# edegens/ptype

Hardware: AMD Instinct MI355X
Metric: messages/sec (higher is better)
Workload: dtype int64; 1 GPU; model=calculator actor (Calculator.Multiply), global_batch=8388608, parallelism=actors sharded over 1 GPU(s), actors=131072, chunks=1, wire=v2, record_bytes=20, reply_bytes=9, client_batch=SoA (actor u32, A i64, B i64), hip_graph=True, steps_per_graph=1, placement=random, delivery=mailbox, mailbox_slots=131072, mailbox_ring_bytes=1344380288, mailbox_record_bytes=8

## Files before the change

### ptype_amd/csrc/hip/mailbox_sort_dev.hpp

```cpp
#pragma once
#include <algorithm>
#include <type_traits>
#include <vector>

#include "mailbox.hpp"
#include "mailbox_dev.hpp"
#include "route_common.hpp"
#include "sort_common.hpp"
#include "tune.hpp"

namespace ptype {

namespace {
constexpr uint32_t kCompactMark = 0x80000000u;
constexpr uint32_t kCompactLong = 0x80000000u;
constexpr int kOrdThreads = 512;
constexpr int kOrdK = 4;
constexpr int kOrdWin = kOrdThreads * kOrdK;
constexpr int kOrdWaves = kOrdThreads / kWave;
constexpr uint32_t kOrdStateMax = 4096;
}

constexpr uint32_t kGroupBlocks = 32;
constexpr uint32_t kNoSlot = 0xffffffffu;
constexpr uint32_t kSpillSlot = 0xfffffffeu;
constexpr uint32_t kRunSpilled = 0x80000000u;

template <int MODE>
__global__ __launch_bounds__(kST) void mbx_count_kernel(SortIn in, uint32_t log_s, uint32_t* __restrict__ hist,
                                                        uint32_t* __restrict__ gsum, uint32_t* __restrict__ rw) {
  __shared__ uint32_t cnt[kMboxSortMaxShards];
  const uint32_t S = 1u << log_s;
  const uint32_t v = virt_block(blockIdx.x, in.G);
  for (uint32_t s = threadIdx.x; s < S; s += kST) cnt[s] = 0;
  __syncthreads();
  const uint32_t t0 = v * in.tpb, t1 = min(t0 + in.tpb, in.tiles);
  uint32_t a[kSK];
  if (t0 < t1) load_actors(in, t0, a);
  for (uint32_t t = t0; t < t1; ++t) {
    int r[kSK];
    uint32_t mb[kSK];
    resolve_k<MODE>(in, a, r, mb);
    if (t + 1 < t1) load_actors(in, t + 1, a);
#pragma unroll
    for (int k = 0; k < kSK; ++k) {
      const int64_t i = tile_index(t, k);
      const bool ok = r[k] == in.rank_self && mb[k] < kMaxMbox;
      if (i < in.M) rw[i] = ok ? mb[k] : kNoSlot;
      if (ok) atomicAdd(&cnt[mb[k] & (S - 1)], 1u);
    }
  }
  __syncthreads();
  uint32_t* g = gsum + (size_t)(v / kGroupBlocks) * S;
  for (uint32_t s = threadIdx.x; s < S; s += kST) {
    const uint32_t c = cnt[s];
    hist[(size_t)v * S + s] = c;
    if (c) atomicAdd(&g[s], c);
  }
}

template <bool A2, bool MC>
__device__ __forceinline__ void load_routed(const SortIn& in, const uint32_t* __restrict__ rw, uint32_t t,
                                            uint32_t (&m)[kSK], int64_t (&x0)[kSK], int64_t (&x1)[kSK],
                                            int64_t (&x2)[kSK], uint32_t (&meth)[kSK]) {
#pragma unroll
  for (int k = 0; k < kSK; ++k) {
    const int64_t i = tile_index(t, k);
    const bool ok = i < in.M;
    m[k] = ok ? __builtin_nontemporal_load(rw + i) : kNoSlot;
    x0[k] = ok ? __builtin_nontemporal_load(in.a0 + i) : 0;
    x1[k] = ok && in.a1 ? __builtin_nontemporal_load(in.a1 + i) : 0;
    x2[k] = 0;
    if constexpr (A2) x2[k] = ok ? __builtin_nontemporal_load(in.a2 + i) : 0;
    meth[k] = in.method_uniform;
    if constexpr (MC) meth[k] = ok ? (uint32_t)in.mcol[i] : 0u;
  }
}

__host__ __device__ constexpr size_t scatter_lds_bytes(uint32_t S) { return (size_t)S * (16 + 4 * (kST / kWave)); }

template <bool A2, bool MC>
__global__ __launch_bounds__(kST) void mbx_scatter_kernel(SortIn in, MboxView mv, const uint32_t* __restrict__ hist,
                                                          const uint32_t* __restrict__ gsum,
                                                          uint32_t* __restrict__ rw,
                                                          uint32_t* __restrict__ sidx, uint32_t* __restrict__ tinfo,
                                                          ReplyView rv, bool spill, bool all_sidx) {
  extern __shared__ __align__(16) unsigned char smem_sc[];
  const uint32_t S = 1u << mv.log_s;
  unsigned long long* base = reinterpret_cast<unsigned long long*>(smem_sc);
  uint32_t* run = reinterpret_cast<uint32_t*>(base + S);
  uint32_t* room = run + S;
  uint32_t* wcnt_all = room + S;
  auto wcnt = [&](unsigned ww, uint32_t sh) -> uint32_t& { return wcnt_all[ww * S + sh]; };
  const uint64_t Q = 1ull << mv.log_q;
  const uint32_t v = virt_block(blockIdx.x, in.G);
  const unsigned w = threadIdx.x / kWave, lane = lane_id();
  const uint32_t g0 = v / kGroupBlocks, v0 = g0 * kGroupBlocks;
  for (uint32_t s = threadIdx.x; s < S; s += kST) {
    uint32_t p = 0;
    for (uint32_t g = 0; g < g0; ++g) p += gsum[(size_t)g * S + s];
    for (uint32_t u = v0; u < v; ++u) p += hist[(size_t)u * S + s];
    run[s] = p;
    const uint64_t tl = *ctr_tail(mv, s), hd = *ctr_head(mv, s);
    base[s] = tl;
    const uint64_t free = hd + Q > tl ? hd + Q - tl : 0;
    room[s] = (uint32_t)(free < 0xffffffffull ? free : 0xffffffffull);
  }
  unsigned long long n_enq = 0, n_ovf = 0, n_miss = 0, n_spill = 0;
  const uint32_t t0 = v * in.tpb, t1 = min(t0 + in.tpb, in.tiles);
  for (uint32_t t = t0; t < t1; ++t) {
    for (uint32_t s = lane; s < S; s += kWave) wcnt(w, s) = 0;
    uint32_t mb[kSK], meth[kSK];
    int64_t v0[kSK], v1[kSK], v2[kSK];
    load_routed<A2, MC>(in, rw, t, mb, v0, v1, v2, meth);
    uint32_t wr[kSK], sh[kSK];
#pragma unroll
    for (int k = 0; k < kSK; ++k) {
      const bool ok = mb[k] != kNoSlot;
      sh[k] = mb[k] & (S - 1);
      const uint64_t peers = match_bits(sh[k], mv.log_s, __ballot(ok));
      const unsigned below = mbcnt64(peers);
      const int leader = peers ? __builtin_ctzll(peers) : 0;
      unsigned old = 0;
      if (ok && below == 0) {
        old = wcnt(w, sh[k]);
        wcnt(w, sh[k]) = old + (unsigned)__popcll(peers);
      }
      wr[k] = (unsigned)__shfl((int)old, leader) + below;
    }
    __syncthreads();
    int sp = 0;
    for (uint32_t s = threadIdx.x; s < S; s += kST) {
      uint32_t rr = run[s];
#pragma unroll
      for (int ww = 0; ww < kST / kWave; ++ww) {
        const uint32_t c = wcnt(ww, s);
        wcnt(ww, s) = rr;
        rr += c;
      }
      run[s] = rr;
      sp |= rr > room[s];
    }
    bool tile_spill = false;
    if (spill) tile_spill = __syncthreads_or(sp) != 0;
    else __syncthreads();
    const bool wsidx = all_sidx || tile_spill;
#pragma unroll
    for (int k = 0; k < kSK; ++k) {
      const int64_t i = tile_index(t, k);
      if (i >= in.M) continue;
      const uint32_t origin = in.origin_base + (uint32_t)i;
      if (mb[k] == kNoSlot) {
        ++n_miss;
        if (wsidx) sidx[i] = kNoSlot;
        write_status(rv, origin, kStatusNoActor);
        continue;
      }
      const uint32_t off = wcnt(w, sh[k]) + wr[k];
      if (off >= room[sh[k]]) {
        if (spill) {
          ++n_spill;
          sidx[i] = kSpillSlot;
          continue;
        }
        ++n_ovf;
        if (wsidx) sidx[i] = kNoSlot;
        write_status(rv, origin, kStatusOverflow);
        continue;
      }
      const int64_t x0 = v0[k], x1 = v1[k], x2 = v2[k];
      const uint32_t mt = meth[k];
      const uint64_t slot = slot_at(mv, sh[k], base[sh[k]] + off);
      if (wsidx) sidx[i] = (uint32_t)slot;
      if (mt < 128u && fits_i32(x0) && fits_i32(x1) && x2 == 0) {
        *reinterpret_cast<u32x4*>(rec_a(mv, slot)) =
            u32x4{origin | kCompactMark, mb[k] | (mt << 24), (uint32_t)x0, (uint32_t)x1};
      } else {
        const uint32_t fl = x2 != 0 ? (uint32_t)kFlagA2 : 0u;
        *reinterpret_cast<u32x4*>(rec_a(mv, slot)) =
            u32x4{origin | kCompactMark, mb[k] | kCompactLong, (mt & 0xffffu) | (fl << 16), 0u};
        *reinterpret_cast<u32x4*>(rec_b(mv, slot)) =
            u32x4{(uint32_t)x0, (uint32_t)((uint64_t)x0 >> 32), (uint32_t)x1, (uint32_t)((uint64_t)x1 >> 32)};
        if (fl) mv.a2[slot] = x2;
      }
      ++n_enq;
    }
    if (tinfo) {
      for (uint32_t s = threadIdx.x; s < S; s += kST) {
        const uint32_t r0 = wcnt(0, s), rr = run[s];
        const uint32_t cc = r0 >= room[s] ? 0u : min(rr - r0, room[s] - r0);
        tinfo[(size_t)t * 2 * S + s] = (uint32_t)(base[s] + r0) + shard_rot(mv, s);
        tinfo[(size_t)t * 2 * S + S + s] = cc | (rr > room[s] ? kRunSpilled : 0u);
      }
    }
    __syncthreads();
  }
  block_add_stats(mv.stats, n_enq, kMbEnqueued, n_ovf, kMbOverflow, n_miss, kMbNoActor);
  if (spill) {
    __syncthreads();
    block_add_stats(mv.stats, n_spill, kMbSpilled, 0, -1, 0, -1);
  }
}

__host__ __device__ constexpr size_t onesweep_lds_bytes(uint32_t S) { return (size_t)S * (8 + 4 + 4 + 4 * (kST / kWave)); }

template <bool A2, bool MC, int SK = kSK>
__device__ __forceinline__ void load_cols(const SortIn& in, uint32_t t, int64_t (&v0)[SK], int64_t (&v1)[SK],
                                          int64_t (&v2)[SK], uint32_t (&meth)[SK]) {
#pragma unroll
  for (int k = 0; k < SK; ++k) {
    const int64_t i = tile_index<SK>(t, k);
    const bool ok = i < in.M;
    v0[k] = ok ? __builtin_nontemporal_load(in.a0 + i) : 0;
    v1[k] = ok && in.a1 ? __builtin_nontemporal_load(in.a1 + i) : 0;
    v2[k] = 0;
    if constexpr (A2) v2[k] = ok ? __builtin_nontemporal_load(in.a2 + i) : 0;
    meth[k] = in.method_uniform;
    if constexpr (MC) meth[k] = ok ? (uint32_t)in.mcol[i] : 0u;
  }
}

__device__ __forceinline__ uint32_t bitlen64(uint64_t x) { return x ? 64u - (uint32_t)__clzll(x) : 0u; }
__device__ __forceinline__ uint32_t wave_max_u32(uint32_t v) {
  for (int off = 32; off > 0; off >>= 1) v = max(v, (uint32_t)__shfl_xor((int)v, off));
  return v;
}

__device__ __forceinline__ void rec8_next_from(const uint32_t* r8max, uint32_t* r8w, uint32_t* host, uint32_t tiles);
__device__ __forceinline__ void rec8_next(const SortIn& in, uint32_t* r8w, uint32_t* host, uint32_t tiles) {
  rec8_next_from(in.r8max, r8w, host, tiles);
}
__device__ __forceinline__ void rec8_next_from(const uint32_t* r8max, uint32_t* r8w, uint32_t* host, uint32_t tiles) {
  __shared__ uint32_t mx[3];
  if (threadIdx.x < 3) mx[threadIdx.x] = 0;
  __syncthreads();
  uint32_t bm = 0, b0 = 0, b1 = 0;
  for (uint32_t t = threadIdx.x; t < tiles; t += blockDim.x) {
    const uint32_t x = __hip_atomic_fetch_add(const_cast<uint32_t*>(r8max) + t, 0u, __ATOMIC_RELAXED,
                                              __HIP_MEMORY_SCOPE_AGENT);
    bm = max(bm, x & 0xffu), b0 = max(b0, (x >> 8) & 0xffu), b1 = max(b1, (x >> 16) & 0xffu);
  }
  bm = wave_max_u32(bm), b0 = wave_max_u32(b0), b1 = wave_max_u32(b1);
  if (lane_id() == 0) {
    atomicMax(&mx[0], bm);
    atomicMax(&mx[1], b0);
    atomicMax(&mx[2], b1);
  }
  __syncthreads();
  if (threadIdx.x == 0) {
    const uint32_t wm = max(mx[0], 1u), n0 = max(mx[1], 1u), n1 = max(mx[2], 1u);
    uint32_t w = 0;
    if (wm <= 24 && wm + n0 + n1 <= 52) {
      const uint32_t w0 = n0 + (52 - wm - n0 - n1) / 2;
      w = wm | (w0 << 8) | ((52 - wm - w0) << 16);
    } else {
      const uint32_t wmc = min(wm, 24u), w0 = (52 - wmc) / 2;
      w = wmc | (w0 << 8) | ((52 - wmc - w0) << 16) | 0x80000000u;
    }
    *r8w = w;
    if (host) __hip_atomic_store(host, w, __ATOMIC_RELAXED, __HIP_MEMORY_SCOPE_SYSTEM);
  }
}

constexpr uint32_t kPresMax = 1u << 18;
__host__ __device__ constexpr uint32_t pres_words(uint32_t n_dir) { return ((n_dir + 15) / 16 + 3) & ~3u; }
template <int = 0>
__global__ __launch_bounds__(256) void mbx_presence_kernel(const uint8_t* __restrict__ dirr, uint32_t n_dir,
                                                           int rank_self, uint32_t* __restrict__ pres) {
  const uint32_t wi = blockIdx.x * 256u + threadIdx.x;
  if (wi >= pres_words(n_dir)) return;
  alignas(16) uint8_t b[16];
  if (wi * 16 + 16 <= n_dir) {
    *reinterpret_cast<uint4*>(b) = *reinterpret_cast<const uint4*>(dirr + (size_t)wi * 16);
  } else {
#pragma unroll
    for (uint32_t j = 0; j < 16; ++j) b[j] = wi * 16 + j < n_dir ? dirr[wi * 16 + j] : kRankMissing;
  }
  uint32_t w = 0;
#pragma unroll
  for (uint32_t j = 0; j < 16; ++j) {
    const uint32_t st = b[j] == (uint8_t)rank_self ? 1u : b[j] == kRankFallback ? 2u : 0u;
    w |= st << (2 * j);
  }
  pres[wi] = w;
}
__device__ __forceinline__ void stage_pres(const SortIn& in, uint32_t* lpres) {
  const uint32_t nw = pres_words(in.n_dir);
  for (uint32_t w = threadIdx.x * 4; w < nw; w += blockDim.x * 4)
    *reinterpret_cast<uint4*>(lpres + w) = *reinterpret_cast<const uint4*>(in.pres + w);
}
template <int SK>
__device__ __forceinline__ void resolve_pres(const SortIn& in, const uint32_t* lpres, const uint32_t (&a)[SK],
                                             int (&r)[SK], uint32_t (&mb)[SK]) {
#pragma unroll
  for (int k = 0; k < SK; ++k) {
    mb[k] = a[k];
    if (a[k] < in.n_dir) {
      const uint32_t st = (lpres[a[k] >> 4] >> ((a[k] & 15) * 2)) & 3u;
      r[k] = st == 1 ? in.rank_self : -1;
      if (st == 2) lookup_entry(in.table, in.mask, actor_key(a[k]), r[k], mb[k]);
    } else if (a[k] != 0xffffffffu) {
      lookup_entry(in.table, in.mask, actor_key(a[k]), r[k], mb[k]);
    } else {
      r[k] = -1;
    }
  }
}

template <int MODE, int SK>
__device__ __forceinline__ void os_resolve(const SortIn& in, const uint32_t* lpres, const uint32_t (&a)[SK], int (&r)[SK],
                                           uint32_t (&mb)[SK]) {
  if constexpr (MODE == 4) resolve_pres<SK>(in, lpres, a, r, mb);
  else resolve_k<MODE, SK>(in, a, r, mb);
}

template <int SK>
__device__ __forceinline__ void os_rank(const SortIn& in, uint32_t log_s, uint32_t t, const int (&r)[SK],
                                        uint32_t (&mb)[SK], uint32_t* wrow, uint32_t (&wr)[SK]) {
  const uint32_t S = 1u << log_s;
#pragma unroll
  for (int k = 0; k < SK; ++k) {
    const bool ok = tile_index<SK>(t, k) < in.M && r[k] == in.rank_self && mb[k] < kMaxMbox;
    if (!ok) mb[k] = kNoSlot;
    const uint32_t sh = mb[k] & (S - 1);
    const uint64_t peers = match_bits(sh, log_s, __ballot(ok));
    const unsigned below = mbcnt64(peers);
    const int leader = peers ? __builtin_ctzll(peers) : 0;
    unsigned old = 0;
    if (ok && below == 0) {
      old = wrow[sh];
      wrow[sh] = old + (unsigned)__popcll(peers);
    }
    wr[k] = (unsigned)__shfl((int)old, leader) + below;
  }
}

__device__ __forceinline__ uint32_t os_wave_offsets(uint32_t* wcnt_all, uint32_t S, uint32_t s) {
  uint32_t c = 0;
#pragma unroll
  for (int ww = 0; ww < kST / kWave; ++ww) {
    const uint32_t x = wcnt_all[ww * S + s];
    wcnt_all[ww * S + s] = c;
    c += x;
  }
  return c;
}
__device__ __forceinline__ uint32_t os_reserve(const MboxView& mv, uint32_t s, uint32_t c) {
  return c ? atomicAdd(&mv.resv[s * kResvStride], c) : 0u;
}
__device__ __forceinline__ uint32_t os_ring_room(const MboxView& mv, uint32_t s, uint64_t& tl) {
  const uint64_t Q = 1ull << mv.log_q;
  tl = *ctr_tail(mv, s);
  const uint64_t hd = *ctr_head(mv, s);
  const uint64_t free = hd + Q > tl ? hd + Q - tl : 0;
  return (uint32_t)(free < 0xffffffffull ? free : 0xffffffffull);
}
__device__ __forceinline__ int os_run_info(const MboxView& mv, uint32_t* __restrict__ tinfo, uint32_t t, uint32_t S,
                                           uint32_t s, uint64_t tl, uint32_t rm, uint64_t excl, uint32_t c) {
  if (tinfo) {
    const uint32_t cc = excl >= rm ? 0u : (uint32_t)min((uint64_t)c, rm - excl);
    tinfo[(size_t)t * 2 * S + s] = (uint32_t)(tl + excl) + shard_rot(mv, s);
    tinfo[(size_t)t * 2 * S + S + s] = cc | (excl + c > rm ? kRunSpilled : 0u);
  }
  return excl + c > rm;
}

template <int SK>
__device__ __forceinline__ uint32_t os_fields(const SortIn& in, uint32_t w8, const uint32_t (&mb)[SK],
                                              const int64_t (&v0)[SK], const int64_t (&v1)[SK], uint32_t* tmax) {
  uint32_t escm = 0;
  if (!(in.rec8 || in.recw)) return escm;
  uint64_t or_m = 0, or_0 = 0, or_1 = 0;
  const uint32_t wm = w8 & 0xffu, w0 = (w8 >> 8) & 0xffu, w1 = (w8 >> 16) & 0xffu;
#pragma unroll
  for (int k = 0; k < SK; ++k) {
    if (mb[k] == kNoSlot) continue;
    const uint64_t z0 = ((uint64_t)v0[k] << 1) ^ (uint64_t)(v0[k] >> 63);
    const uint64_t z1 = ((uint64_t)v1[k] << 1) ^ (uint64_t)(v1[k] >> 63);
    or_m |= mb[k], or_0 |= z0, or_1 |= z1;
    if (in.rec8 && ((mb[k] >> wm) != 0 || (z0 >> w0) != 0 || (z1 >> w1) != 0)) escm |= 1u << k;
  }
  const uint32_t bm = wave_max_u32(bitlen64(or_m)), b0 = wave_max_u32(bitlen64(or_0)),
                 b1 = wave_max_u32(bitlen64(or_1));
  if (lane_id() == 0) {
    atomicMax(&tmax[0], bm);
    atomicMax(&tmax[1], b0);
    atomicMax(&tmax[2], b1);
  }
  return escm;
}

template <int SK>
struct PackedRanks {
  uint32_t p[SK / 2];
  __device__ __forceinline__ uint32_t operator[](int k) const { return (p[k >> 1] >> ((k & 1) * 16)) & 0xffffu; }
};

template <int SK, typename CT>
__device__ __forceinline__ void os_store_msg(const SortIn& in, const MboxView& mv, const ReplyView& rv, int64_t i,
                                             const unsigned long long* base, const uint32_t* room, const uint32_t* pre,
                                             const uint32_t* wrow, uint32_t mbk, uint32_t wrk, int64_t x0, int64_t x1,
                                             int64_t x2, uint32_t mt, bool esc, uint32_t w8, bool spill, bool wsidx,
                                             uint32_t* __restrict__ sidx, uint32_t* __restrict__ rw, CT& n_enq, CT& n_ovf,
                                             CT& n_miss, CT& n_spill) {
  const uint32_t S = 1u << mv.log_s;
  const uint32_t origin = in.origin_base + (uint32_t)i;
  if (mbk == kNoSlot) {
    ++n_miss;
    if (wsidx) sidx[i] = kNoSlot;
    write_status(rv, origin, kStatusNoActor);
    return;
  }
  const uint32_t sh = mbk & (S - 1);
  const uint32_t off = pre[sh] + wrow[sh] + wrk;
  if (off >= room[sh] || (esc && spill)) {
    if (spill) {
      ++n_spill;
      sidx[i] = kSpillSlot;
      rw[i] = mbk;
      return;
    }
    ++n_ovf;
    if (wsidx) sidx[i] = kNoSlot;
    write_status(rv, origin, kStatusOverflow);
    return;
  }
  const uint64_t slot = slot_at(mv, sh, base[sh] + off);
  if (wsidx) sidx[i] = (uint32_t)slot;
  if (in.recw) {
    *reinterpret_cast<u32x4*>(rec_a(mv, slot)) =
        u32x4{(uint32_t)x0, (uint32_t)((uint64_t)x0 >> 32), (uint32_t)x1, (uint32_t)((uint64_t)x1 >> 32)};
    rec_place(mv)[slot] = (uint16_t)(i & ((kST * SK) - 1));
  } else if (in.rec8 && esc) {
    reinterpret_cast<uint64_t*>(mv.rec)[slot] = (uint64_t)(i & ((kST * SK) - 1)) | (1ull << 63);
    *reinterpret_cast<u32x4*>(in.r8esc + 2 * slot) =
        u32x4{(uint32_t)x0, (uint32_t)((uint64_t)x0 >> 32), mbk, 0u};
  } else if (in.rec8) {
    const uint32_t wm = w8 & 0xffu, w0 = (w8 >> 8) & 0xffu;
    const uint64_t z0 = ((uint64_t)x0 << 1) ^ (uint64_t)(x0 >> 63);
    const uint64_t z1 = ((uint64_t)x1 << 1) ^ (uint64_t)(x1 >> 63);
    reinterpret_cast<uint64_t*>(mv.rec)[slot] =
        (uint64_t)(i & ((kST * SK) - 1)) | ((uint64_t)mbk << 12) | (z0 << (12 + wm)) | (z1 << (12 + wm + w0));
  } else if (mt < 128u && fits_i32(x0) && fits_i32(x1) && x2 == 0) {
    *reinterpret_cast<u32x4*>(rec_a(mv, slot)) =
        u32x4{origin | kCompactMark, mbk | (mt << 24), (uint32_t)x0, (uint32_t)x1};
  } else {
    const uint32_t fl = x2 != 0 ? (uint32_t)kFlagA2 : 0u;
    *reinterpret_cast<u32x4*>(rec_a(mv, slot)) =
        u32x4{origin | kCompactMark, mbk | kCompactLong, (mt & 0xffffu) | (fl << 16), 0u};
    *reinterpret_cast<u32x4*>(rec_b(mv, slot)) =
        u32x4{(uint32_t)x0, (uint32_t)((uint64_t)x0 >> 32), (uint32_t)x1, (uint32_t)((uint64_t)x1 >> 32)};
    if (fl) mv.a2[slot] = x2;
  }
  ++n_enq;
}

template <int MODE, bool A2, bool MC, int SK = kSK>
__device__ __forceinline__ uint32_t onesweep_tile(const SortIn& in, const MboxView& mv, unsigned long long* __restrict__ desc,
                                                  unsigned* __restrict__ tctr, uint32_t* __restrict__ gsum,
                                                  uint32_t* __restrict__ sidx, uint32_t* __restrict__ tinfo,
                                                  uint32_t* __restrict__ rw, const ReplyView& rv, bool spill,
                                                  bool all_sidx, unsigned char* smem_os, bool reserve = false) {
  const uint32_t S = 1u << mv.log_s;
  unsigned long long* base = reinterpret_cast<unsigned long long*>(smem_os);
  uint32_t* room = reinterpret_cast<uint32_t*>(base + S);
  uint32_t* pre = room + S;
  uint32_t* wcnt_all = pre + S;
  auto wcnt = [&](unsigned ww, uint32_t sh) -> uint32_t& { return wcnt_all[ww * S + sh]; };
  __shared__ uint32_t tile_s;
  __shared__ uint32_t tmax[3];
  const unsigned w = threadIdx.x / kWave, lane = lane_id();
  if (threadIdx.x < 3) tmax[threadIdx.x] = 0;
  const uint32_t tag = epoch_tag(tctr[1]);
  if (threadIdx.x == 0 && !reserve) {
    const uint32_t t = atomicAdd(&tctr[0], 1u);
    if (t == in.tiles - 1) atomicExch(&tctr[0], 0u);
    tile_s = t;
  }
  for (uint32_t s = lane; s < S; s += kWave) wcnt(w, s) = 0;
  uint32_t* lpres = reinterpret_cast<uint32_t*>(smem_os + ((onesweep_lds_bytes(S) + 15) & ~(size_t)15));
  if constexpr (MODE == 4) stage_pres(in, lpres);
  __syncthreads();
  const uint32_t t = reserve ? virt_block(blockIdx.x, gridDim.x) : tile_s;
  uint32_t a[SK], mb[SK], meth[SK];
  int64_t v0[SK], v1[SK], v2[SK];
  int r[SK];
  load_actors<SK>(in, t, a);
  load_cols<A2, MC, SK>(in, t, v0, v1, v2, meth);
  os_resolve<MODE, SK>(in, lpres, a, r, mb);
  uint32_t wr[SK];
  os_rank<SK>(in, mv.log_s, t, r, mb, wcnt_all + w * S, wr);
  __syncthreads();
  unsigned long long timeouts = 0;
  int sp = 0;
  for (uint32_t s = threadIdx.x; s < S; s += kST) {
    uint64_t excl = 0;
    unsigned long long* d = desc + (size_t)t * S + s;
    const uint32_t c = os_wave_offsets(wcnt_all, S, s);
    if (reserve) {
      excl = os_reserve(mv, s, c);
    } else if (t == 0) {
      __hip_atomic_exchange(d, desc_word(tag, kDescP, c), __ATOMIC_RELAXED, __HIP_MEMORY_SCOPE_AGENT);
    } else {
      __hip_atomic_exchange(d, desc_word(tag, kDescA, c), __ATOMIC_RELAXED, __HIP_MEMORY_SCOPE_AGENT);
      excl = lookback(desc + s, S, (int64_t)t - 1, tag, timeouts);
      __hip_atomic_exchange(d, desc_word(tag, kDescP, excl + c), __ATOMIC_RELAXED, __HIP_MEMORY_SCOPE_AGENT);
    }
    if (!reserve && t == in.tiles - 1) gsum[s] = (uint32_t)(excl + c);
    uint64_t tl;
    const uint32_t rm = os_ring_room(mv, s, tl);
    base[s] = tl;
    room[s] = rm;
    pre[s] = (uint32_t)excl;
    sp |= os_run_info(mv, tinfo, t, S, s, tl, rm, excl, c);
  }
  const uint32_t w8 = in.rec8 ? *in.r8w : 0u;
  const bool maxima = in.rec8 || in.recw;
  const uint32_t escm = os_fields<SK>(in, w8, mb, v0, v1, tmax);
  sp |= escm != 0;
  bool tile_spill = false;
  if (spill) tile_spill = __syncthreads_or(sp) != 0;
  else __syncthreads();
  if (tile_spill && tinfo && threadIdx.x == 0) tinfo[(size_t)t * 2 * S + S] |= kRunSpilled;
  const bool wsidx = all_sidx || tile_spill;
  unsigned long long n_enq = 0, n_ovf = 0, n_miss = 0, n_spill = 0;
#pragma unroll
  for (int k = 0; k < SK; ++k) {
    const int64_t i = tile_index<SK>(t, k);
    if (i >= in.M) continue;
    os_store_msg<SK>(in, mv, rv, i, base, room, pre, wcnt_all + w * S, mb[k], wr[k], v0[k], v1[k], v2[k], meth[k],
                     (escm >> k) & 1u, w8, spill, wsidx, sidx, rw, n_enq, n_ovf, n_miss, n_spill);
  }
  if (maxima && threadIdx.x == 0) (void)atomicExch(&in.r8max[t], tmax[0] | (tmax[1] << 8) | (tmax[2] << 16));
  block_add_stats(mv.stats, n_enq, kMbEnqueued, n_ovf, kMbOverflow, n_miss, kMbNoActor);
  __syncthreads();
  block_add_stats(mv.stats, n_spill, kMbSpilled, timeouts, kMbLookback, 0, -1);
  return t;
}

template <int MODE, bool A2, bool MC>
__global__ __launch_bounds__(kST) void mbx_onesweep_kernel(SortIn in, MboxView mv, unsigned long long* __restrict__ desc,
                                                           unsigned* __restrict__ tctr, uint32_t* __restrict__ gsum,
                                                           uint32_t* __restrict__ sidx, uint32_t* __restrict__ tinfo,
                                                           uint32_t* __restrict__ rw, ReplyView rv, bool spill,
                                                           bool all_sidx, bool reserve) {
  extern __shared__ __align__(16) unsigned char smem_os[];
  (void)onesweep_tile<MODE, A2, MC>(in, mv, desc, tctr, gsum, sidx, tinfo, rw, rv, spill, all_sidx, smem_os, reserve);
}

__host__ __device__ constexpr size_t persist_lds_bytes(uint32_t S) {
  return (size_t)S * (8 + 4 + 2 * 4 + 2 * 4 * (kST / kWave));
}

template <int = 0>
__global__ __launch_bounds__(kST) void mbx_persist_sort_kernel(SortIn in, MboxView mv, uint32_t* __restrict__ sidx,
                                                               uint32_t* __restrict__ tinfo, uint32_t* __restrict__ rw,
                                                               ReplyView rv) {
  constexpr int SK = kSK;
  extern __shared__ __align__(16) unsigned char smem_ps[];
  const uint32_t S = 1u << mv.log_s;
  unsigned long long* base = reinterpret_cast<unsigned long long*>(smem_ps);
  uint32_t* room = reinterpret_cast<uint32_t*>(base + S);
  uint32_t* pre2 = room + S;
  uint32_t* wcnt2 = pre2 + 2 * S;
  uint32_t* lpres = reinterpret_cast<uint32_t*>(smem_ps + ((persist_lds_bytes(S) + 15) & ~(size_t)15));
  __shared__ uint32_t tmax[3];
  const unsigned w = threadIdx.x / kWave, lane = lane_id();
  const uint32_t G = gridDim.x, T = in.tiles;
  uint32_t first = blockIdx.x, stride = G, n = blockIdx.x < T ? (T - blockIdx.x + G - 1) / G : 0u;
  if (G >= 8 && (G & 7) == 0 && (T & 7) == 0) {
    const uint32_t j = blockIdx.x >> 3, T8 = T >> 3;
    stride = G >> 3;
    first = (blockIdx.x & 7) * T8 + j;
    n = j < T8 ? (T8 - j + stride - 1) / stride : 0u;
  }
  if (n == 0) return;
  stage_pres(in, lpres);
  for (uint32_t s = threadIdx.x; s < S; s += kST) {
    uint64_t tl;
    room[s] = os_ring_room(mv, s, tl);
    base[s] = tl;
  }
  if (threadIdx.x < 3) tmax[threadIdx.x] = 0;
  for (uint32_t s = lane; s < S; s += kWave) wcnt2[w * S + s] = 0;
  __syncthreads();
  const uint32_t w8 = in.rec8 ? *in.r8w : 0u;
  const bool maxima = in.rec8 || in.recw;
  uint32_t n_enq = 0, n_ovf = 0, n_miss = 0, n_spill = 0;
  uint32_t nx[SK];
  PackedRanks<SK> wrp;
  {
    uint32_t a[SK], wr[SK];
    int r[SK];
    load_actors<SK>(in, first, a);
    os_resolve<4, SK>(in, lpres, a, r, nx);
    os_rank<SK>(in, mv.log_s, first, r, nx, wcnt2 + w * S, wr);
#pragma unroll
    for (int k = 0; k < SK / 2; ++k) wrp.p[k] = wr[2 * k] | (wr[2 * k + 1] << 16);
  }
  __syncthreads();
  uint32_t rc = 0, rx = 0;
  if (threadIdx.x < S) {
    rc = os_wave_offsets(wcnt2, S, threadIdx.x);
    rx = os_reserve(mv, threadIdx.x, rc);
  }
  for (uint32_t it = 0; it < n; ++it) {
    const uint32_t t = first + it * stride, b = it & 1;
    uint32_t* pre = pre2 + b * S;
    uint32_t* wcnt_all = wcnt2 + b * (kST / kWave) * S;
    uint32_t mb[SK], meth[SK];
    int64_t v0[SK], v1[SK], v2[SK];
#pragma unroll
    for (int k = 0; k < SK; ++k) mb[k] = nx[k];
    load_cols<false, false, SK>(in, t, v0, v1, v2, meth);
    const bool more = it + 1 < n;
    if (more) load_actors<SK>(in, t + stride, nx);
    int sp = 0;
    if (threadIdx.x < S) {
      const uint32_t s = threadIdx.x;
      pre[s] = rx;
      sp = os_run_info(mv, tinfo, t, S, s, base[s], room[s], rx, rc);
    }
    const uint32_t escm = os_fields<SK>(in, w8, mb, v0, v1, tmax);
    sp |= escm != 0;
    const bool tile_spill = __syncthreads_or(sp) != 0;
    if (threadIdx.x == 0) {
      if (tile_spill) tinfo[(size_t)t * 2 * S + S] |= kRunSpilled;
      if (maxima) {
        (void)atomicExch(&in.r8max[t], tmax[0] | (tmax[1] << 8) | (tmax[2] << 16));
        tmax[0] = tmax[1] = tmax[2] = 0;
      }
    }
#pragma unroll
    for (int k = 0; k < SK; ++k) {
      const int64_t i = tile_index<SK>(t, k);
      if (i >= in.M) continue;
      os_store_msg<SK>(in, mv, rv, i, base, room, pre, wcnt_all + w * S, mb[k], wrp[k], v0[k], v1[k], v2[k], meth[k],
                       (escm >> k) & 1u, w8, true, tile_spill, sidx, rw, n_enq, n_ovf, n_miss, n_spill);
    }
    if (more) {
      uint32_t* wnext = wcnt2 + (b ^ 1) * (kST / kWave) * S;
      for (uint32_t s = lane; s < S; s += kWave) wnext[w * S + s] = 0;
      uint32_t a[SK], wr[SK];
      int r[SK];
#pragma unroll
      for (int k = 0; k < SK; ++k) a[k] = nx[k];
      os_resolve<4, SK>(in, lpres, a, r, nx);
      os_rank<SK>(in, mv.log_s, t + stride, r, nx, wnext + w * S, wr);
#pragma unroll
      for (int k = 0; k < SK / 2; ++k) wrp.p[k] = wr[2 * k] | (wr[2 * k + 1] << 16);
      __syncthreads();
      if (threadIdx.x < S) {
        rc = os_wave_offsets(wnext, S, threadIdx.x);
        rx = os_reserve(mv, threadIdx.x, rc);
      }
    }
  }
  block_add_stats(mv.stats, n_enq, kMbEnqueued, n_ovf, kMbOverflow, n_miss, kMbNoActor);
  __syncthreads();
  block_add_stats(mv.stats, n_spill, kMbSpilled, 0, -1, 0, -1);
}

struct SortRec {
  uint32_t origin, mb, method, flags;
  int64_t a0, a1, a2;
  bool valid;
};

__device__ __forceinline__ bool rec_is_long(const u32x4& ha) { return (ha.y & kCompactLong) != 0; }

__device__ __forceinline__ SortRec decode_sorted(const u32x4& ha, const u32x4& hb, int64_t a2v) {
  SortRec x;
  x.valid = (ha.x & kCompactMark) != 0;
  x.origin = ha.x & ~kCompactMark;
  if (!rec_is_long(ha)) {
    x.mb = ha.y & 0xffffffu;
    x.method = (ha.y >> 24) & 0x7fu;
    x.flags = 0;
    x.a0 = (int64_t)(int32_t)ha.z;
    x.a1 = (int64_t)(int32_t)ha.w;
    x.a2 = 0;
  } else {
    x.mb = ha.y & 0xffffffu;
    x.method = ha.z & 0xffffu;
    x.flags = ha.z >> 16;
    x.a0 = (int64_t)(((uint64_t)hb.y << 32) | hb.x);
    x.a1 = (int64_t)(((uint64_t)hb.w << 32) | hb.z);
    x.a2 = (x.flags & kFlagA2) ? a2v : 0;
  }
  return x;
}

template <bool FRESH, int SK = kSK>
__device__ __forceinline__ SortRec decode_rec8(uint64_t r, const SortIn& in, uint32_t w8, uint32_t tile_origin) {
  const uint32_t wm = w8 & 0xffu, w0 = (w8 >> 8) & 0xffu, w1 = (w8 >> 16) & 0xffu;
  const uint64_t m0 = (1ull << w0) - 1;
  SortRec x;
  x.valid = true;
  x.origin = tile_origin + (uint32_t)(r & ((kST * SK) - 1));
  x.mb = (uint32_t)((r >> 12) & ((1ull << wm) - 1));
  x.method = in.method_uniform;
  x.flags = 0;
  x.a2 = 0;
  const uint64_t z0 = (r >> (12 + wm)) & m0, z1 = (r >> (12 + wm + w0)) & ((1ull << w1) - 1);
  x.a0 = (int64_t)(z0 >> 1) ^ -(int64_t)(z0 & 1);
  x.a1 = (int64_t)(z1 >> 1) ^ -(int64_t)(z1 & 1);
  return x;
}

__device__ __forceinline__ SortRec decode_wide(const u32x4& h, const SortIn& in, uint32_t origin) {
  SortRec x;
  x.valid = true;
  x.origin = origin;
  x.mb = 0;
  x.method = in.method_uniform;
  x.flags = 0;
  x.a0 = (int64_t)(((uint64_t)h.y << 32) | h.x);
  x.a1 = (int64_t)(((uint64_t)h.w << 32) | h.z);
  x.a2 = 0;
  return x;
}

__device__ __forceinline__ SortRec load_sorted(const MboxView& mv, uint64_t slot) {
  const u32x4 ha = *reinterpret_cast<const u32x4*>(rec_a(mv, slot));
  u32x4 hb = {0u, 0u, 0u, 0u};
  int64_t a2v = 0;
  if (rec_is_long(ha)) {
    hb = *reinterpret_cast<const u32x4*>(rec_b(mv, slot));
    if (((ha.z >> 16) & kFlagA2) && mv.a2) a2v = mv.a2[slot];
  }
  return decode_sorted(ha, hb, a2v);
}

__device__ __forceinline__ uint32_t epoch_total(uint32_t* gsum, uint32_t ngroups, uint32_t S, uint32_t s, bool clear) {
  uint32_t t = 0;
  for (uint32_t g = 0; g < ngroups; ++g) {
    t += gsum[(size_t)g * S + s];
    if (clear) gsum[(size_t)g * S + s] = 0u;
  }
  return t;
}

__device__ __forceinline__ uint32_t epoch_sum(const MboxView& mv, uint32_t* gsum, uint32_t ngroups, uint32_t S,
                                              uint32_t s) {
  return mv.resv ? atomicExch(&mv.resv[s * kResvStride], 0u) : epoch_total(gsum, ngroups, S, s, true);
}

__device__ __forceinline__ void epoch_commit(const MboxView& mv, uint32_t s, uint32_t tot) {
  const uint64_t t = *ctr_tail(mv, s) + tot;
  *ctr_tail(mv, s) = t;
  *ctr_done(mv, s) = t;
  *ctr_head(mv, s) = t;
}

template <int FIXED, bool FRESH = false, int RF = 0, int SK = kSK>
__device__ __forceinline__ void drain_tile_msg(MboxView mv, SortIn in, uint32_t t,
                                               const uint32_t* __restrict__ sidx, const uint32_t* __restrict__ rw,
                                               int64_t* __restrict__ state, uint32_t n_state, uint64_t delay_ticks,
                                               OutboxView ob, ReplyView rv, unsigned long long& done,
                                               unsigned long long& failed, unsigned long long& holes) {
  uint32_t sl[SK];
#pragma unroll
  for (int k = 0; k < SK; ++k) {
    const int64_t i = tile_index<SK>(t, k);
    sl[k] = i < in.M ? __builtin_nontemporal_load(sidx + i) : kNoSlot;
  }
  using RecT = typename std::conditional<RF == 1, uint64_t, u32x4>::type;
  const uint32_t w8 = RF == 1 ? *in.r8w : 0u;
  RecT ha[SK];
#pragma unroll
  for (int k = 0; k < SK; ++k) {
    if constexpr (RF == 1) {
      const uint64_t* rp = reinterpret_cast<const uint64_t*>(mv.rec) + (sl[k] < kSpillSlot ? sl[k] : 0);
      ha[k] = sl[k] < kSpillSlot ? (FRESH ? __builtin_nontemporal_load(rp) : *rp) : 0ull;
    } else {
      const u32x4* rp = reinterpret_cast<const u32x4*>(rec_a(mv, sl[k] < kSpillSlot ? sl[k] : 0));
      ha[k] = sl[k] < kSpillSlot ? (FRESH ? __builtin_nontemporal_load(rp) : *rp) : u32x4{0u, 0u, 0u, 0u};
    }
  }
#pragma unroll
  for (int k = 0; k < SK; ++k) {
    if (sl[k] == kNoSlot) continue;
    SortRec x;
    if (sl[k] == kSpillSlot) {
      const int64_t i = tile_index<SK>(t, k);
      x.valid = true;
      x.mb = rw[i];
      x.method = in.mcol ? (uint32_t)in.mcol[i] : in.method_uniform;
      x.flags = 0;
      x.a0 = in.a0[i];
      x.a1 = in.a1 ? in.a1[i] : 0;
      x.a2 = in.a2 ? in.a2[i] : 0;
    } else if constexpr (RF == 1) {
      x = decode_rec8<FRESH, SK>(ha[k], in, w8, in.origin_base + t * (kST * SK));
    } else if constexpr (RF == 2) {
      x = decode_wide(ha[k], in, 0u);
    } else {
      u32x4 hb = {0u, 0u, 0u, 0u};
      int64_t a2v = 0;
      if (rec_is_long(ha[k])) {
        const u32x4* bp = reinterpret_cast<const u32x4*>(rec_b(mv, sl[k]));
        hb = FRESH ? __builtin_nontemporal_load(bp) : *bp;
        if (((ha[k].z >> 16) & kFlagA2) && mv.a2) a2v = FRESH ? __builtin_nontemporal_load(mv.a2 + sl[k]) : mv.a2[sl[k]];
      }
// ... 31 lines not shown
    drain_tile_msg<FIXED>(mv, in, t, sidx, rw, state, n_state, delay_ticks, ob, rv, done, failed, holes);
  block_add_stats(mv.stats, done, kMbProcessed, failed, kMbFailed, holes, kMbHoles);
  __shared__ bool last;
  if (threadIdx.x == 0) last = last_block_ticket(ticket);
  __syncthreads();
  if (last) {
    const uint32_t S = 1u << mv.log_s;
    for (uint32_t s = threadIdx.x; s < S; s += kST) epoch_commit(mv, s, epoch_sum(mv, gsum, ngroups, S, s));
    if (threadIdx.x == 0) tctr[1] += 1u;
  }
}

template <typename OwnT>
struct RunLds {
  uint32_t* bias;
  uint32_t* excl;
  OwnT* owner;
};

template <typename OwnT>
__device__ __forceinline__ uint32_t load_tile_runs(const MboxView& mv, const uint32_t* __restrict__ tinfo, uint32_t t,
                                                   const RunLds<OwnT>& L, int& spill) {
  __shared__ uint32_t wsum[kST / kWave];
  __shared__ uint32_t total_s;
  const uint32_t S = 1u << mv.log_s;
  const unsigned w = threadIdx.x / kWave, lane = lane_id();
  const uint32_t per = (S + kST - 1) / kST, s0 = threadIdx.x * per, s1 = min(S, s0 + per);
  uint32_t cnt[2] = {0u, 0u};
  uint32_t mine = 0;
  int sp = 0;
  for (uint32_t s = s0, q = 0; s < s1; ++s, ++q) {
    const uint32_t cw = tinfo[(size_t)t * 2 * S + S + s];
    sp |= (cw & kRunSpilled) != 0;
    cnt[q] = cw & ~kRunSpilled;
    mine += cnt[q];
    L.bias[s] = tinfo[(size_t)t * 2 * S + s];
  }
  const uint32_t incl = wave_incl_scan(mine);
  if (lane == kWave - 1) wsum[w] = incl;
  spill = __syncthreads_or(sp);
  uint32_t acc = incl - mine;
  for (unsigned ww = 0; ww < w; ++ww) acc += wsum[ww];
  if (threadIdx.x == kST - 1) total_s = acc + mine;
  for (uint32_t s = s0, q = 0; s < s1; ++s, ++q) {
    L.excl[s] = acc;
    L.bias[s] -= acc;
    for (uint32_t j = acc; j < acc + cnt[q]; ++j) L.owner[j] = (OwnT)s;
    acc += cnt[q];
  }
  __syncthreads();
  return total_s;
}

constexpr uint8_t kAbsent = 0xff;
__host__ __device__ constexpr size_t ring_drain_lds_bytes(uint32_t S, size_t tile = kSTile) {
  return S <= 256 ? tile * (8 + 1) + (size_t)S * 8 : tile * (8 + 2 + 1) + (size_t)S * 8;
}

struct DrainCounts {
  unsigned long long done = 0, failed = 0, holes = 0;
};

template <int FIXED, bool NARROW, bool FRESH, int RF = 0, int SK = kSK>
__device__ __forceinline__ DrainCounts drain_ring_tile(MboxView mv, SortIn in, uint32_t t,
                                                       const uint32_t* __restrict__ tinfo,
                                                       const uint32_t* __restrict__ sidx,
                                                       const uint32_t* __restrict__ rw, int64_t* __restrict__ state,
                                                       uint32_t n_state, uint64_t delay_ticks, OutboxView ob,
                                                       ReplyView rv, unsigned char* smem_rd) {
  unsigned long long done = 0, failed = 0, holes = 0;
  using OwnT = typename std::conditional<NARROW, uint8_t, uint16_t>::type;
  const uint32_t S = 1u << mv.log_s;
  int64_t* sval = reinterpret_cast<int64_t*>(smem_rd);
  RunLds<OwnT> L;
  L.bias = reinterpret_cast<uint32_t*>(sval + (kST * SK));
  L.excl = L.bias + S;
  L.owner = reinterpret_cast<OwnT*>(L.excl + S);
  uint8_t* sst = NARROW ? reinterpret_cast<uint8_t*>(L.owner) : reinterpret_cast<uint8_t*>(L.owner + (kST * SK));
  const uint64_t i0 = (uint64_t)t * (kST * SK);
  const uint32_t n_t = (uint32_t)min((uint64_t)(kST * SK), (uint64_t)in.M - i0);
  if constexpr (!NARROW)
    for (uint32_t j = threadIdx.x; j < (kST * SK); j += kST) sst[j] = kAbsent;
  int spill = 0;
  const uint32_t T = load_tile_runs(mv, tinfo, t, L, spill);
  if (spill) {
    drain_tile_msg<FIXED, FRESH, RF, SK>(mv, in, t, sidx, rw, state, n_state, delay_ticks, ob, rv, done, failed, holes);
    return DrainCounts{done, failed, holes};
  }
  const uint64_t sbase_mask = (1ull << mv.log_q) - 1;
  using RecT = typename std::conditional<RF == 1, uint64_t, u32x4>::type;
  const uint32_t w8 = RF == 1 ? *in.r8w : 0u;
  RecT ha[SK];
  uint32_t sl[SK];
  uint16_t pl[SK];
#pragma unroll
  for (int k = 0; k < SK; ++k) {
    const uint32_t j = (uint32_t)k * kST + threadIdx.x;
    sl[k] = kNoSlot;
    if (j < T) {
      const uint32_t s = L.owner[j];
      sl[k] = (uint32_t)(((uint64_t)s << mv.log_q) | ((L.bias[s] + j) & sbase_mask));
      if constexpr (RF == 1) {
        const uint64_t* rp = reinterpret_cast<const uint64_t*>(mv.rec) + sl[k];
        ha[k] = FRESH ? __builtin_nontemporal_load(rp) : *rp;
      } else {
        const u32x4* rp = reinterpret_cast<const u32x4*>(rec_a(mv, sl[k]));
        ha[k] = FRESH ? __builtin_nontemporal_load(rp) : *rp;
        if constexpr (RF == 2) {
          const uint16_t* pp = rec_place(mv) + sl[k];
          pl[k] = FRESH ? __builtin_nontemporal_load(pp) : *pp;
        }
      }
    }
  }
  if constexpr (NARROW) {
    __syncthreads();
    for (uint32_t j = threadIdx.x; j < (kST * SK); j += kST) sst[j] = kAbsent;
    __syncthreads();
  }
#pragma unroll
  for (int k = 0; k < SK; ++k) {
    if (sl[k] == kNoSlot) continue;
    SortRec x;
    if constexpr (RF == 1) {
      x = decode_rec8<FRESH, SK>(ha[k], in, w8, in.origin_base + (uint32_t)i0);
    } else if constexpr (RF == 2) {
      x = decode_wide(ha[k], in, in.origin_base + (uint32_t)i0 + pl[k]);
    } else {
      u32x4 hb = {0u, 0u, 0u, 0u};
      int64_t a2v = 0;
      if (rec_is_long(ha[k])) {
        const u32x4* bp = reinterpret_cast<const u32x4*>(rec_b(mv, sl[k]));
        hb = FRESH ? __builtin_nontemporal_load(bp) : *bp;
        if (((ha[k].z >> 16) & kFlagA2) && mv.a2) a2v = FRESH ? __builtin_nontemporal_load(mv.a2 + sl[k]) : mv.a2[sl[k]];
      }
      x = decode_sorted(ha[k], hb, a2v);
    }
    const uint32_t local = x.origin - in.origin_base - (uint32_t)i0;
    if (!x.valid || local >= n_t) {
      ++holes;
      continue;
    }
    MsgRecord m;
    m.actor = x.mb;
    m.method = (uint16_t)(FIXED ? FIXED : x.method);
    m.flags = (uint16_t)x.flags;
    m.a0 = x.a0, m.a1 = x.a1, m.a2 = x.a2;
    const ReplyRecord rr = run_handler(m, state, n_state, delay_ticks, ob);
    failed += rr.status != kStatusOk;
    sval[local] = rr.value;
    sst[local] = (uint8_t)rr.status;
    ++done;
  }
  __syncthreads();
#pragma unroll
  for (int k = 0; k < SK; ++k) {
    const uint32_t j = (uint32_t)k * kST + threadIdx.x;
    if (j < n_t && sst[j] != kAbsent) put_reply_nt(rv, in.origin_base + (uint32_t)(i0 + j), sval[j], sst[j]);
  }
  return DrainCounts{done, failed, holes};
}

template <int FIXED, bool NARROW, int RF, int SK = kSK>
__global__ __launch_bounds__(kST, (NARROW && FIXED) ? 8 : 1) void mbx_drain_ring_kernel(MboxView mv, SortIn in, const uint32_t* __restrict__ tinfo,
                                                             const uint32_t* __restrict__ sidx,
                                                             const uint32_t* __restrict__ rw,
                                                             int64_t* __restrict__ state, uint32_t n_state,
                                                             uint64_t delay_ticks, OutboxView ob, ReplyView rv,
                                                             uint32_t* __restrict__ gsum, uint32_t ngroups,
                                                             unsigned* __restrict__ ticket, unsigned* __restrict__ tctr,
                                                             uint32_t* __restrict__ r8host) {
  extern __shared__ __align__(16) unsigned char smem_rd[];
  const uint32_t S = 1u << mv.log_s;
  DrainCounts dc;
  const uint32_t t = virt_block(blockIdx.x, gridDim.x);
  if (t < in.tiles)
    dc = drain_ring_tile<FIXED, NARROW, false, RF, SK>(mv, in, t, tinfo, sidx, rw, state, n_state, delay_ticks, ob,
                                                       rv, smem_rd);
  block_add_stats(mv.stats, dc.done, kMbProcessed, dc.failed, kMbFailed, dc.holes, kMbHoles);
  __shared__ bool last;
  if (threadIdx.x == 0) last = last_block_ticket(ticket);
  __syncthreads();
  if (last) {
    for (uint32_t s = threadIdx.x; s < S; s += kST) epoch_commit(mv, s, epoch_sum(mv, gsum, ngroups, S, s));
    if (threadIdx.x == 0) tctr[1] += 1u;
    if constexpr (RF != 0) rec8_next(in, const_cast<uint32_t*>(in.r8w), r8host, in.tiles);
  }
}

template <int MODE, bool A2, bool MC, int FIXED, int RF, int SK = kSK>
__global__ __launch_bounds__(kST) void mbx_sortdrain_kernel(SortIn in, MboxView mv, unsigned long long* __restrict__ desc,
                                                            unsigned* __restrict__ tctr, uint32_t* __restrict__ gsum,
                                                            uint32_t* __restrict__ sidx, uint32_t* __restrict__ tinfo,
                                                            uint32_t* __restrict__ rw, ReplyView rv,
                                                            int64_t* __restrict__ state, uint32_t n_state,
                                                            uint64_t delay_ticks, OutboxView ob,
                                                            unsigned* __restrict__ ticket, bool reserve,
                                                            uint32_t* __restrict__ r8host) {
  extern __shared__ __align__(16) unsigned char smem_sd[];
  const uint32_t S = 1u << mv.log_s;
  const uint32_t t = onesweep_tile<MODE, A2, MC, SK>(in, mv, desc, tctr, gsum, sidx, tinfo, rw, rv, true, false,
                                                     smem_sd, reserve);
  asm volatile("s_waitcnt vmcnt(0)" ::: "memory");
  __syncthreads();
  const DrainCounts dc = drain_ring_tile<FIXED, true, true, RF, SK>(mv, in, t, tinfo, sidx, rw, state, n_state,
                                                                    delay_ticks, ob, rv, smem_sd);
  block_add_stats(mv.stats, dc.done, kMbProcessed, dc.failed, kMbFailed, dc.holes, kMbHoles);
  __shared__ bool last;
  if (threadIdx.x == 0) {
    if (t == in.tiles - 1) __builtin_amdgcn_fence(__ATOMIC_RELEASE, "agent");
    last = last_block_ticket(ticket);
    if (last) __builtin_amdgcn_fence(__ATOMIC_ACQUIRE, "agent");
  }
  __syncthreads();
  if (last) {
    for (uint32_t s = threadIdx.x; s < S; s += kST)
      epoch_commit(mv, s, epoch_sum(mv, gsum, 1, S, s));
    if (threadIdx.x == 0) tctr[1] += 1u;
    if constexpr (RF != 0) rec8_next(in, const_cast<uint32_t*>(in.r8w), r8host, in.tiles);
  }
}

__device__ __forceinline__ bool arrival_fits(const MboxView& mv, const SortIn& in, uint32_t t, uint64_t& pos0,
                                             uint32_t tile = kSTile) {
  const uint32_t s = t & ((1u << mv.log_s) - 1);
  const uint64_t Q = 1ull << mv.log_q;
  const uint64_t tl = *ctr_tail(mv, s), hd = *ctr_head(mv, s);
  const uint64_t room = hd + Q > tl ? hd + Q - tl : 0;
  const uint64_t off = (uint64_t)(t >> mv.log_s) * tile;
  const uint64_t n_t = min((uint64_t)tile, (uint64_t)in.M - (uint64_t)t * tile);
  pos0 = tl + off;
  return off + n_t <= room;
}

template <int MODE, bool A2, bool MC>
__global__ __launch_bounds__(kST) void mbx_arrival_enqueue_kernel(SortIn in, MboxView mv, ReplyView rv) {
  unsigned long long n_enq = 0, n_miss = 0, n_spill = 0;
  const uint32_t t = virt_block(blockIdx.x, gridDim.x);
  if (t < in.tiles) {
    uint64_t pos0 = 0;
    const bool fits = arrival_fits(mv, in, t, pos0);
    const uint32_t s = t & ((1u << mv.log_s) - 1);
    uint32_t a[kSK], mb[kSK], meth[kSK];
    int64_t x0[kSK], x1[kSK], x2[kSK];
    int r[kSK];
#pragma unroll
    for (int k = 0; k < kSK; ++k) {
      const int64_t i = tile_index(t, k);
      const bool ok = i < in.M;
      a[k] = ok ? __builtin_nontemporal_load(in.actor + i) : 0xffffffffu;
      x0[k] = ok ? __builtin_nontemporal_load(in.a0 + i) : 0;
      x1[k] = ok && in.a1 ? __builtin_nontemporal_load(in.a1 + i) : 0;
      x2[k] = 0;
      if constexpr (A2) x2[k] = ok ? __builtin_nontemporal_load(in.a2 + i) : 0;
      meth[k] = in.method_uniform;
      if constexpr (MC) meth[k] = ok ? (uint32_t)in.mcol[i] : 0u;
    }
    resolve_k<MODE>(in, a, r, mb);
#pragma unroll
    for (int k = 0; k < kSK; ++k) {
      const int64_t i = tile_index(t, k);
      if (i >= in.M) continue;
      const uint32_t origin = in.origin_base + (uint32_t)i;
      const bool ok = r[k] == in.rank_self && mb[k] < kMaxMbox;
      const uint64_t slot = slot_at(mv, s, pos0 + (uint64_t)(i - (int64_t)t * kSTile));
      if (!ok) {
        ++n_miss;
        write_status(rv, origin, kStatusNoActor);
        if (fits) *reinterpret_cast<u32x4*>(rec_a(mv, slot)) = u32x4{0u, 0u, 0u, 0u};
        continue;
      }
      if (!fits) {
        ++n_spill;
        continue;
      }
      const uint32_t mt = meth[k];
      if (mt < 128u && fits_i32(x0[k]) && fits_i32(x1[k]) && x2[k] == 0) {
        *reinterpret_cast<u32x4*>(rec_a(mv, slot)) =
            u32x4{origin | kCompactMark, mb[k] | (mt << 24), (uint32_t)x0[k], (uint32_t)x1[k]};
      } else {
        const uint32_t fl = x2[k] != 0 ? (uint32_t)kFlagA2 : 0u;
        *reinterpret_cast<u32x4*>(rec_a(mv, slot)) =
            u32x4{origin | kCompactMark, mb[k] | kCompactLong, (mt & 0xffffu) | (fl << 16), 0u};
        *reinterpret_cast<u32x4*>(rec_b(mv, slot)) = u32x4{(uint32_t)x0[k], (uint32_t)((uint64_t)x0[k] >> 32),
                                                           (uint32_t)x1[k], (uint32_t)((uint64_t)x1[k] >> 32)};
        if (fl) mv.a2[slot] = x2[k];
      }
      ++n_enq;
    }
  }
  block_add_stats(mv.stats, n_enq, kMbEnqueued, n_miss, kMbNoActor, n_spill, kMbSpilled);
}

template <int FIXED, int MODE>
__global__ __launch_bounds__(kST) void mbx_arrival_drain_kernel(MboxView mv, SortIn in, int64_t* __restrict__ state,
                                                                uint32_t n_state, uint64_t delay_ticks, OutboxView ob,
                                                                ReplyView rv, unsigned* __restrict__ ticket) {
  unsigned long long done = 0, failed = 0;
  const uint32_t S = 1u << mv.log_s;
  const uint32_t t = virt_block(blockIdx.x, gridDim.x);
  if (t < in.tiles) {
    uint64_t pos0 = 0;
    const bool fits = arrival_fits(mv, in, t, pos0);
    const uint32_t s = t & (S - 1);
    SortRec x[kSK];
    if (fits) {
      u32x4 ha[kSK];
#pragma unroll
      for (int k = 0; k < kSK; ++k) {
        const int64_t i = tile_index(t, k);
        ha[k] = i < in.M ? *reinterpret_cast<const u32x4*>(rec_a(mv, slot_at(mv, s, pos0 + (uint64_t)(i - (int64_t)t * kSTile))))
// ... 547 lines not shown
```

Baseline: 61.95 billion msg/s.

## Prefetch next tile's argument columns and restructure spill vote and reply stores

The persistent sort kernel now loads the next tile's A/B argument columns during the current tile's store phase, so global loads overlap with work. Full tiles take an unguarded load path and skip the per-element bounds check. The block-wide spill reduction uses a wave __any plus a double-buffered LDS vote instead of __syncthreads_or. The drain reply path batches its LDS reads before issuing the nontemporal stores and adds an explicit vmcnt wait. These changes raise register pressure and add fragile inline asm and waitcnt constants.

After: 65.14 billion msg/s (median of 6 runs). 5.1% higher.

```diff
diff --git a/ptype_amd/csrc/hip/mailbox_sort_dev.hpp b/ptype_amd/csrc/hip/mailbox_sort_dev.hpp
--- a/ptype_amd/csrc/hip/mailbox_sort_dev.hpp
+++ b/ptype_amd/csrc/hip/mailbox_sort_dev.hpp
@@ -25,6 +25,7 @@
 constexpr uint32_t kNoSlot = 0xffffffffu;
 constexpr uint32_t kSpillSlot = 0xfffffffeu;
 constexpr uint32_t kRunSpilled = 0x80000000u;
+constexpr int kWaitVmcnt0 = 0x0f70;
 
 template <int MODE>
 __global__ __launch_bounds__(kST) void mbx_count_kernel(SortIn in, uint32_t log_s, uint32_t* __restrict__ hist,
@@ -220,6 +221,28 @@
   }
 }
 
+template <int SK>
+__device__ __forceinline__ bool tile_is_full(const SortIn& in, uint32_t t) {
+  return in.a1 != nullptr && ((int64_t)t + 1) * (kST * SK) <= (int64_t)in.M;
+}
+template <int SK>
+__device__ __forceinline__ void load_args_tile(const SortIn& in, uint32_t t, bool full, int64_t (&v0)[SK],
+                                               int64_t (&v1)[SK]) {
+  if (full) {
+#pragma unroll
+    for (int k = 0; k < SK; ++k) {
+      const int64_t i = tile_index<SK>(t, k);
+      v0[k] = __builtin_nontemporal_load(in.a0 + i);
+      v1[k] = __builtin_nontemporal_load(in.a1 + i);
+    }
+    __builtin_amdgcn_sched_barrier(0);
+  } else {
+    int64_t v2[SK];
+    uint32_t meth[SK];
+    load_cols<false, false, SK>(in, t, v0, v1, v2, meth);
+  }
+}
+
 __device__ __forceinline__ uint32_t bitlen64(uint64_t x) { return x ? 64u - (uint32_t)__clzll(x) : 0u; }
 __device__ __forceinline__ uint32_t wave_max_u32(uint32_t v) {
   for (int off = 32; off > 0; off >>= 1) v = max(v, (uint32_t)__shfl_xor((int)v, off));
@@ -388,6 +411,12 @@
     atomicMax(&tmax[2], b1);
   }
   return escm;
+}
+
+template <int SK>
+__device__ __forceinline__ void os_loads_in(const int64_t (&v0)[SK], const int64_t (&v1)[SK], const uint32_t (&nx)[SK]) {
+#pragma unroll
+  for (int k = 0; k < SK; ++k) asm volatile("" ::"v"(v0[k]), "v"(v1[k]), "v"(nx[k]));
 }
 
 template <int SK>
@@ -565,6 +594,7 @@
   uint32_t* wcnt2 = pre2 + 2 * S;
   uint32_t* lpres = reinterpret_cast<uint32_t*>(smem_ps + ((persist_lds_bytes(S) + 15) & ~(size_t)15));
   __shared__ uint32_t tmax[3];
+  __shared__ uint32_t vote[2];
   const unsigned w = threadIdx.x / kWave, lane = lane_id();
   const uint32_t G = gridDim.x, T = in.tiles;
   uint32_t first = blockIdx.x, stride = G, n = blockIdx.x < T ? (T - blockIdx.x + G - 1) / G : 0u;
@@ -582,17 +612,21 @@
     base[s] = tl;
   }
   if (threadIdx.x < 3) tmax[threadIdx.x] = 0;
+  if (threadIdx.x < 2) vote[threadIdx.x] = 0;
   for (uint32_t s = lane; s < S; s += kWave) wcnt2[w * S + s] = 0;
   __syncthreads();
   const uint32_t w8 = in.rec8 ? *in.r8w : 0u;
   const bool maxima = in.rec8 || in.recw;
   uint32_t n_enq = 0, n_ovf = 0, n_miss = 0, n_spill = 0;
   uint32_t nx[SK];
+  int64_t v0[SK], v1[SK];
   PackedRanks<SK> wrp;
   {
     uint32_t a[SK], wr[SK];
     int r[SK];
+    const bool full = tile_is_full<SK>(in, first);
     load_actors<SK>(in, first, a);
+    load_args_tile<SK>(in, first, full, v0, v1);
     os_resolve<4, SK>(in, lpres, a, r, nx);
     os_rank<SK>(in, mv.log_s, first, r, nx, wcnt2 + w * S, wr);
 #pragma unroll
@@ -608,13 +642,14 @@
     const uint32_t t = first + it * stride, b = it & 1;
     uint32_t* pre = pre2 + b * S;
     uint32_t* wcnt_all = wcnt2 + b * (kST / kWave) * S;
-    uint32_t mb[SK], meth[SK];
-    int64_t v0[SK], v1[SK], v2[SK];
+    const bool full = tile_is_full<SK>(in, t);
+    uint32_t mb[SK];
 #pragma unroll
     for (int k = 0; k < SK; ++k) mb[k] = nx[k];
-    load_cols<false, false, SK>(in, t, v0, v1, v2, meth);
     const bool more = it + 1 < n;
+    const bool full_next = more && tile_is_full<SK>(in, t + stride);
     if (more) load_actors<SK>(in, t + stride, nx);
+    os_loads_in<SK>(v0, v1, nx);
     int sp = 0;
     if (threadIdx.x < S) {
       const uint32_t s = threadIdx.x;
@@ -623,7 +658,9 @@
     }
     const uint32_t escm = os_fields<SK>(in, w8, mb, v0, v1, tmax);
     sp |= escm != 0;
-    const bool tile_spill = __syncthreads_or(sp) != 0;
+    if (__any(sp) && lane == 0) vote[b] = 1u;
+    __syncthreads();
+    const bool tile_spill = __builtin_amdgcn_readfirstlane((int)vote[b]) != 0;
     if (threadIdx.x == 0) {
       if (tile_spill) tinfo[(size_t)t * 2 * S + S] |= kRunSpilled;
       if (maxima) {
@@ -634,11 +671,12 @@
 #pragma unroll
     for (int k = 0; k < SK; ++k) {
       const int64_t i = tile_index<SK>(t, k);
-      if (i >= in.M) continue;
-      os_store_msg<SK>(in, mv, rv, i, base, room, pre, wcnt_all + w * S, mb[k], wrp[k], v0[k], v1[k], v2[k], meth[k],
+      if (!full && i >= in.M) continue;
+      os_store_msg<SK>(in, mv, rv, i, base, room, pre, wcnt_all + w * S, mb[k], wrp[k], v0[k], v1[k], 0, in.method_uniform,
                        (escm >> k) & 1u, w8, true, tile_spill, sidx, rw, n_enq, n_ovf, n_miss, n_spill);
     }
     if (more) {
+      load_args_tile<SK>(in, t + stride, full_next, v0, v1);
       uint32_t* wnext = wcnt2 + (b ^ 1) * (kST / kWave) * S;
       for (uint32_t s = lane; s < S; s += kWave) wnext[w * S + s] = 0;
       uint32_t a[SK], wr[SK];
@@ -650,6 +688,7 @@
 #pragma unroll
       for (int k = 0; k < SK / 2; ++k) wrp.p[k] = wr[2 * k] | (wr[2 * k + 1] << 16);
       __syncthreads();
+      if (threadIdx.x == 0) vote[b] = 0u;
       if (threadIdx.x < S) {
         rc = os_wave_offsets(wnext, S, threadIdx.x);
         rx = os_reserve(mv, threadIdx.x, rc);
@@ -987,11 +1026,20 @@
     sst[local] = (uint8_t)rr.status;
     ++done;
   }
-  __syncthreads();
+  __builtin_amdgcn_s_waitcnt(kWaitVmcnt0);
+  __syncthreads();
+  uint8_t rst[SK];
+  int64_t rval[SK];
 #pragma unroll
   for (int k = 0; k < SK; ++k) {
     const uint32_t j = (uint32_t)k * kST + threadIdx.x;
-    if (j < n_t && sst[j] != kAbsent) put_reply_nt(rv, in.origin_base + (uint32_t)(i0 + j), sval[j], sst[j]);
+    rst[k] = j < n_t ? sst[j] : kAbsent;
+    rval[k] = sval[j];
+  }
+#pragma unroll
+  for (int k = 0; k < SK; ++k) {
+    const uint32_t j = (uint32_t)k * kST + threadIdx.x;
+    if (rst[k] != kAbsent) put_reply_nt(rv, in.origin_base + (uint32_t)(i0 + j), rval[k], rst[k]);
   }
   return DrainCounts{done, failed, holes};
 }
```
